# AlwinEsch/pvr.rtl.radiofm

Measured on AMD Instinct MI355X. Metric: IQ MS/s demodulated (whole node) + achieved HBM GB/s on FIR stage, higher is better.
Workload: dtype f32

## Files before the change

### pvr.rtl.radiofm_amd/csrc/fmd_batch.hip

```cpp
#include "../../include/fmd.h"

#include <hip/hip_runtime.h>
#include <hip/hip_ext.h>

#include <algorithm>
#include <chrono>
#include <cmath>
#include <cstdio>
#include <cstdlib>
#include <cstring>
#include <deque>
#include <functional>
#include <map>
#include <memory>
#include <mutex>
#include <string>
#include <utility>
#include <vector>

#include "fmd_design.hpp"
#include "fmd_groups.hpp"
#include "fmd_kernels.hip.h"
#include "fmd_receiver.hpp"

// ... 127 lines not shown
  unsigned min_samples = 0;
  int streams_sharing = 0;
  unsigned cpc = 1;
  unsigned Mmax = 0, Mstride = 0, Amax = 0, Rmax = 0;
  std::vector<unsigned> hb_nmax;
  unsigned lastM = 0, lastA = 0, lastR = 0;

  DevBuf<float2> lut, hist[2], demod[2], br[2], mix[2], rdsraw[2], rlpf[2], rs[2], alp[2];
  std::vector<DevBuf<float2>> hbbuf;
  DevBuf<float> if_coeff, rs_coeff, rds_lpf_taps, mf_taps2, audio_taps, ktab;
  DevBuf<float> rpll, rmf, tap_sync;
  DevBuf<double> sctab, sctab256;
  DevBuf<int> pidx;
  static constexpr unsigned kBrFront = 32;
  float2* brp(int q) const { return br[q].p + size_t(kBrFront) * CP; }
  unsigned rs_margin = 0, rs_row = 0;
  int rsr_R = 0, rsr_NW = 0;
  unsigned rsr_nbr = 0, rsr_nbm = 0;
  int rsr_rb = 0;
  DevBuf<float> rsr_tab;
  DevBuf<int> rsr_head, rsr_steps;
  int rsr_mode = -1;
  int n_cus = 256;
  struct HbfPlan
  {
    unsigned n_in = 0, S = 0;
    DevBuf<fmd::HbStep> steps;
    DevBuf<int> seg_first;
  };
  std::vector<std::unique_ptr<HbfPlan>> hbf_plans;
  DevBuf<float2> hbf_tail1, hbf_tail2;
  int hbf_mode = -1;
  static constexpr unsigned kOscH = 64;
  DevBuf<float2> osc_tab[4];
  HostBuf<float2> h_osc;
  Event osc_ev[8];
  bool osc_ev_used[8] = {};
  size_t h_osc_stride = 0;
  float osc_re = 1.0f, osc_im = 0.0f;
  bool osc_on = false;
  int dbg_nomix = 1;
  int dbg_fir_nt = 0;
  int dbg_serial_claim = 0;
  int dbg_hb4 = 1, dbg_ring4 = 1;
  int dbg_fir_ro = 2;
  int dbg_lpf_late = -1;
  double host_ms[4] = {0, 0, 0, 0};
  unsigned host_calls = 0;
  DevBuf<long long> serial_probe;
  int dbg_stage_mask = 63;
  DevBuf<float> fstate;
  DevBuf<int> istate;
  DevBuf<uint16_t> r_data;
  static constexpr int NSLOT = 8;
  static_assert(NSLOT == 8, "osc_ev / osc_ev_used above");
  DevBuf<fmd::RdsGroupRec> queue[NSLOT];
  DevBuf<unsigned> queue_counts;
  unsigned* qcount(int q) const { return queue_counts.p + q; }
  uint32_t drained_call[NSLOT] = {};
  HostBuf<unsigned> h_counts;
  HostBuf<fmd::RdsGroupRec> h_recs;
  unsigned queue_cap = 0;
  Event ev_drained[NSLOT];
  bool drained_pending[NSLOT] = {};
  static constexpr unsigned kExportCursors = 16;
  DevBuf<unsigned> export_cursor;
  unsigned export_seq = 0;
  fmd::ChannelState st{};
  std::vector<fmd::HbCoef> hbcoef;

  DevBuf<float> h_iq, h_audio;
  DevBuf<unsigned long long> pcm_clip;

  std::vector<std::unique_ptr<fmd::GroupDecoder>> gdec;

  int profiling = 0;
  int write_taps = 0;

  int concurrency = 1;
  hipStream_t s_fir = nullptr, s_ser = nullptr, s_post = nullptr, s_rds = nullptr, s_lpf = nullptr;
  struct LightJob
  {
    unsigned R = 0, A = 0, mf_g = 0, alpf_g = 0;
    unsigned rds_lpf_g = 0;
    const unsigned* org = nullptr;
    int q = 0, es = 0, sq = 0;
    bool events = true;
    bool lpf_here = false;
    int audio_after = -1;
    bool status_after_rds = false;
    hipEvent_t prev_aud = nullptr;
    uint32_t call_index = 0;
    void* d_audio = nullptr;
    int pcm = 0;
    size_t audio_stride = 0;
    hipEvent_t tl0 = nullptr, tl1 = nullptr;
  };
  std::vector<std::unique_ptr<fmd_batch>> subs;
  std::vector<unsigned> sub_ch0;
  bool owns_streams = true;
  hipEvent_t vheavy[2] = {nullptr, nullptr};
  hipEvent_t sched_prev2 = nullptr;
// ... 306 lines not shown
      independent = us < 250.0;
      for (int i = 0; i < have; i++)
        (void)hipStreamSynchronize(out[i]);
      (void)hipStreamSynchronize(nullptr);
    }
    if (independent)
      out[have++] = cand;
    else
      rejected.push_back(cand);
  }
  *n_sharing = 0;
  while (have < n && !rejected.empty())
  {
    out[have++] = rejected.back();
    rejected.pop_back();
    ++*n_sharing;
  }
  for (hipStream_t s : rejected)
    (void)hipStreamDestroy(s);
  return have == n ? 0 : -1;
}

fmd_batch::HbfPlan* hbf_plan(fmd_batch* b, unsigned n_in, unsigned S)
{
  for (auto& pl : b->hbf_plans)
    if (pl->n_in == n_in && pl->S == S)
      return pl.get();
  const fmd::Design& d = b->des;
  const int L1H = d.hb[1].len - 1, L2H = d.hb[2].len - 1, RING = fmd::HBF_RING;
  const int n0 = int(n_in + 1) / 2, n1 = (n0 + 1) / 2, n2 = (n1 + 1) / 2;
  std::vector<fmd::HbStep> steps;
  std::vector<int> first;
  const int per = (n2 + int(S) - 1) / int(S);
  for (int a = 0; a < n2; a += per)
  {
    first.push_back(int(steps.size()));
    const int e = std::min(n2, a + per);
    const bool last = e == n2;
    const int need1 = last ? n1 : 2 * (e - 1) + 1, need0 = last ? n0 : 2 * (need1 - 1) + 1;
    int d2 = a, d1 = std::max(0, 2 * a - L2H), d0 = std::max(0, 2 * d1 - L1H);
    while (d2 < e || d1 < need1 || d0 < need0)
    {
      const int a_hi = std::max(d0, std::min({d0 + 16, need0, 2 * d1 - L1H + RING}));
      const int b_hi = std::max(d1, std::min({d1 + 8, need1, a_hi > 0 ? (a_hi - 1) / 2 + 1 : 0, 2 * d2 - L2H + RING}));
      const int c_hi = std::max(d2, std::min({d2 + 4, e, b_hi > 0 ? (b_hi - 1) / 2 + 1 : 0}));
      if (a_hi == d0 && b_hi == d1 && c_hi == d2)
        return nullptr;
      steps.push_back(fmd::HbStep{d0, a_hi - d0, d1, b_hi - d1, d2, c_hi - d2, 0, 0});
      d0 = a_hi;
      d1 = b_hi;
      d2 = c_hi;
    }
    while ((steps.size() - size_t(first.back())) % 4)
      steps.push_back(fmd::HbStep{d0, 0, d1, 0, d2, 0, 0, 0});
  }
  first.push_back(int(steps.size()));
  std::unique_ptr<fmd_batch::HbfPlan> pl(new fmd_batch::HbfPlan);
  pl->n_in = n_in;
  pl->S = unsigned(first.size() - 1);
  if (pl->steps.alloc(steps.size()) || pl->seg_first.alloc(first.size()) ||
      upload(pl->steps.p, steps.data(), steps.size() * sizeof(fmd::HbStep)) ||
      upload(pl->seg_first.p, first.data(), first.size() * sizeof(int)))
    return nullptr;
  if (b->hbf_plans.size() >= 16)
  {
    (void)hipDeviceSynchronize();
    b->hbf_plans.erase(b->hbf_plans.begin());
  }
  b->hbf_plans.push_back(std::move(pl));
  return b->hbf_plans.back().get();
}

bool rsr_configure(fmd_batch* b, int form)
{
  static const int forms[3][2] = {{2, 8}, {4, 4}, {2, 4}};
  const fmd::Design& d = b->des;
  const int R = forms[form][0], NW = forms[form][1];
  const double step = double(d.rs_step);
  const unsigned per_step = unsigned(NW * R);
  const unsigned span = d.rs_order + 1u + unsigned(std::ceil((per_step - 1) * step)) + 1u;
  const unsigned nbr = (span - 1u + 7u) / 8u + 2u;
  const unsigned new_rows = unsigned(std::ceil(per_step * step)) + 8u;
  b->rsr_R = 0;
  if (nbr > 39u || new_rows > unsigned(fmd::RSR_ROWS))
    return false;
  b->rsr_R = R;
  b->rsr_NW = NW;
// ... 129 lines not shown
      auto t = fmd::make_tuner_lut(d.table_size, b->shifts[c]);
      std::copy(t.begin(), t.end(), &lut[size_t(2) * d.table_size * c]);
    }
  }

  b->Mmax = (FMD_MAX_BLOCK + d.D - 1) / d.D + 1;
  b->Mstride = (b->Mmax + 15u) & ~15u;
  b->Amax = unsigned(double(b->Mmax) / double(d.rs_step)) + 4;
  {
    unsigned n = b->Mmax;
    for (size_t s = 0; s < d.hb.size(); s++)
    {
      b->hb_nmax.push_back(n);
      n = (n + 1) / 2;
    }
    b->Rmax = n;
  }
  const unsigned T_lpf = unsigned(d.rds_lpf_taps.size());
  const unsigned T_mf = unsigned(d.rds_mf_taps.size());
  const unsigned T_alp = unsigned(d.lpf_taps.size());

  if (size_t(b->Mstride) * C * sizeof(float2) + 4096 >= (size_t(1) << 32) ||
      size_t(b->Mmax) * CP * sizeof(float2) >= (size_t(1) << 32))
    return fail(FMD_ERR_ARG, "too many channels for one batch at this sample rate (4 GB per row buffer): split the batch");
  int bad = 0;
  bad |= b->lut.alloc(size_t(d.table_size) * C);
  bad |= b->hist[0].alloc(size_t(d.if_order) * C);
  bad |= b->hist[1].alloc(size_t(d.if_order) * C);
  bad |= b->demod[0].alloc(size_t(b->Mstride) * C + fmd::DS);
  bad |= b->demod[1].alloc(size_t(b->Mstride) * C + fmd::DS);
  bad |= b->if_coeff.alloc(d.if_coeff.size() + 64);
  bad |= b->rs_coeff.alloc(d.rs_coeff.size());
  static_assert(fmd_batch::kBrFront >= 2 * fmd::RS_B, "front rows of br");
  bad |= b->br[0].alloc(size_t(fmd_batch::kBrFront + d.rs_order + b->Mmax + 8) * CP);
  bad |= b->br[1].alloc(size_t(fmd_batch::kBrFront + d.rs_order + b->Mmax + 8) * CP);
  if (d.hb.empty())
    return fail(FMD_ERR_ARG, "baseband rate too low for the RDS decimation chain");
  bad |= b->mix[0].alloc(size_t(d.hb[0].len - 1 + b->Mmax) * CP);
  bad |= b->mix[1].alloc(size_t(d.hb[0].len - 1 + b->Mmax) * CP);
  b->hbbuf.resize(d.hb.size() - 1);
  for (size_t s = 1; s < d.hb.size(); s++)
    bad |= b->hbbuf[s - 1].alloc(size_t(d.hb[s].len - 1 + b->hb_nmax[s]) * CP);
  if (d.hb.size() == 3)
  {
    bad |= b->hbf_tail1.alloc(size_t(d.hb[1].len - 1) * CP);
    bad |= b->hbf_tail2.alloc(size_t(d.hb[2].len - 1) * CP);
    for (auto& t : b->osc_tab)
      bad |= t.alloc(size_t(fmd_batch::kOscH) + b->Mmax + 8);
    b->h_osc_stride = size_t(fmd_batch::kOscH) + b->Mmax + 8;
    bad |= b->h_osc.alloc(fmd_batch::NSLOT * b->h_osc_stride);
    for (auto& e : b->osc_ev)
      bad |= e.create() != hipSuccess;
    const int h0 = (d.hb[0].len - 1) / 2, h1 = (d.hb[1].len - 1) / 2, h2 = (d.hb[2].len - 1) / 2;
    const bool chain_kind = h0 == 7 && ((h1 == 11 && h2 == 21) || (h1 == 9 && h2 == 17));
    b->osc_on = chain_kind && CP / 64 >= 64 && d.hb[0].len - 1 <= int(fmd_batch::kOscH);
  }
  bad |= b->rdsraw[0].alloc(size_t(T_lpf - 1 + b->Rmax) * CP);
  bad |= b->rdsraw[1].alloc(size_t(T_lpf - 1 + b->Rmax) * CP);
  bad |= b->rlpf[0].alloc(size_t(b->Rmax) * CP);
  bad |= b->rlpf[1].alloc(size_t(b->Rmax) * CP);
  bad |= b->rpll.alloc(size_t(T_mf - 1 + b->Rmax) * CP);
  bad |= b->rmf.alloc(size_t(b->Rmax) * CP);
  bad |= b->tap_sync.alloc(size_t(b->Rmax) * CP);
  bad |= b->rs[0].alloc(size_t(T_alp - 1 + b->Amax) * CP);
  bad |= b->rs[1].alloc(size_t(T_alp - 1 + b->Amax) * CP);
  bad |= b->alp[0].alloc(size_t(b->Amax) * CP);
  bad |= b->alp[1].alloc(size_t(b->Amax) * CP);
  bad |= b->rds_lpf_taps.alloc(T_lpf);
  bad |= b->mf_taps2.alloc(size_t(2) * T_mf);
  bad |= b->audio_taps.alloc(2 * size_t(T_alp));
  b->rs_margin = fmd::rs_table_margin(d.rs_step);
  b->rs_row = d.rs_order + 1 + 2 * b->rs_margin;
  bad |= b->ktab.alloc(size_t(b->Amax) * b->rs_row + 64);
  bad |= b->pidx.alloc(b->Amax);
  {
    hipDeviceProp_t prop{};
    if (hipGetDeviceProperties(&prop, device) == hipSuccess && prop.multiProcessorCount > 0)
      b->n_cus = prop.multiProcessorCount;
    size_t tab_floats = 0, head_ints = 0, step_ints = 0;
    for (int form = 0; form < 3; form++)
      if (rsr_configure(b.get(), form))
// ... 28 lines not shown
  }
  bad |= b->sctab.alloc(d.sincos_tab.size());
  bad |= b->sctab256.alloc(d.sincos_tab256.size());
  bad |= b->fstate.alloc(size_t(fmd::F_SLOTS) * CP);
  bad |= b->pcm_clip.alloc(CP);
  bad |= b->istate.alloc(size_t(fmd::I_SLOTS) * CP);
  bad |= b->r_data.alloc(size_t(4) * CP);
  b->queue_cap = std::max(4096u, 8u * C);
  for (int q = 0; q < fmd_batch::NSLOT; q++)
    bad |= b->queue[q].alloc(b->queue_cap);
  bad |= b->queue_counts.alloc(fmd_batch::NSLOT);
  bad |= b->h_counts.alloc(fmd_batch::NSLOT);
  bad |= b->export_cursor.alloc(fmd_batch::kExportCursors);
  if (bad)
    return fail(FMD_ERR_DEVICE, std::string("device allocation failed: ") + hipGetErrorString(hipGetLastError()));

  bad |= upload(b->lut.p, lut.data(), lut.size() * sizeof(float));
  bad |= upload(b->if_coeff.p, d.if_coeff.data(), d.if_coeff.size() * sizeof(float));
  bad |= upload(b->rs_coeff.p, d.rs_coeff.data(), d.rs_coeff.size() * sizeof(float));
  bad |= upload(b->rds_lpf_taps.p, d.rds_lpf_taps.data(), T_lpf * sizeof(float));
  bad |= upload(b->audio_taps.p, d.lpf_taps.data(), T_alp * sizeof(float));
  bad |= upload(b->audio_taps.p + T_alp, d.lpf_taps.data(), T_alp * sizeof(float));
  bad |= upload(b->sctab.p, d.sincos_tab.data(), d.sincos_tab.size() * sizeof(double));
  bad |= upload(b->sctab256.p, d.sincos_tab256.data(), d.sincos_tab256.size() * sizeof(double));
  bad |= upload(b->mf_taps2.p, d.rds_mf_taps.data(), T_mf * sizeof(float));
  for (const auto& h : d.hb)
  {
    fmd::HbCoef hc{};
    for (int i = 0; i < h.len; i++)
      hc.c[i] = h.coef[size_t(i)];
    for (int j = 0; 2 * j < h.len && j < 28; j++)
      hc.e[j] = hc.c[2 * j];
    b->hbcoef.push_back(hc);
  }
  if (b->h_err.alloc(2, hipHostMallocMapped | hipHostMallocCoherent))
    return fail(FMD_ERR_DEVICE, "host-mapped error word allocation failed");
  if (b->h_status.alloc(size_t(fmd::HS_WORDS) * CP, hipHostMallocMapped | hipHostMallocCoherent))
    return fail(FMD_ERR_DEVICE, "host-mapped status snapshot allocation failed");
  if (b->d_status.alloc(size_t(fmd::HS_WORDS) * CP))
    return fail(FMD_ERR_DEVICE, "status record allocation failed");
  if (b->org.alloc(size_t(2) * CP) || b->d_edits.alloc(size_t(fmd_batch::NSLOT) * 2 * C))
    return fail(FMD_ERR_DEVICE, "device allocation of the channel edit state failed");
  if (b->h_edits.alloc(size_t(fmd_batch::NSLOT) * 2 * C))
    return fail(FMD_ERR_DEVICE, "page-locked staging allocation failed");
  for (auto& e : b->edit_ev)
    HIPCHK(e.create());
  bind_state(b.get());
  if (!b->st.err || !b->st.hs)
    return fail(FMD_ERR_DEVICE, "host-mapped memory has no device address");
  bad |= init_signal_state(b.get());
  if (bad)
    return fail(FMD_ERR_DEVICE, "upload of constants failed");
  if (do_reset(b.get()))
    return fail(FMD_ERR_DEVICE, "state reset failed");

  b->gdec.resize(C);
  if (shell)
  {
    b->owns_streams = false;
    b->s_fir = shell->s_fir;
    b->s_ser = shell->s_ser;
    b->s_post = shell->s_post;
    b->s_rds = shell->s_rds;
    b->s_lpf = shell->s_lpf;
    b->streams_sharing = shell->streams_sharing;
  }
// ... 1903 lines not shown
```

### pvr.rtl.radiofm_amd/csrc/fmd_batch_process.inc.hpp

```cpp
namespace
{

fmd::DemodConsts demod_consts(const fmd::Design& d)
{
  fmd::DemodConsts k{};
  k.pll_alpha = d.pll_alpha;
  k.pll_beta = d.pll_beta;
  k.nco_hl = d.nco_hl;
  k.nco_ll = d.nco_ll;
  k.demod_gain = d.demod_gain;
  k.p_minfreq = d.p_minfreq;
  k.p_maxfreq = d.p_maxfreq;
  k.p_b0 = d.p_b0;
  k.p_a1 = d.p_a1;
  k.p_a2 = d.p_a2;
  k.p_lf_b0 = d.p_lf_b0;
  k.p_lf_b1 = d.p_lf_b1;
  k.p_minsignal = d.p_minsignal;
  k.p_lock_delay = d.p_lock_delay;
  k.osc_cos = d.rds_osc_cos;
  k.osc_sin = d.rds_osc_sin;
  return k;
}

// ... 310 lines not shown
    }
    evset = &b->ev[size_t(b->prof_calls) * (ST_COUNT + 1)];
  }
  auto timed = [&](int i) -> hipEvent_t { return evset && b->profiling == 1 && !serial_mode ? evset[i].e : nullptr; };
  auto mark = [&](int i) {
    if (evset && b->profiling >= 2 && i > 1)
      note(hipEventRecord(evset[i], sF));
  };

  bool hb_all_normal = d.hb.size() <= 3;
  for (size_t s = 0; s < d.hb.size(); s++)
    hb_all_normal = hb_all_normal && hb_mode[s] == HB_NORMAL && d.hb[s].len != 11 && !d.hb[s].cic;
  fmd_batch::HbfPlan* hbf_pl = nullptr;
  int hbf_kind = -1;
  if (hb_all_normal && d.hb.size() == 3 && b->hbf_mode != 0 && (b->hbf_mode == 1 || CP / 64 >= 64))
  {
    const int h0 = (d.hb[0].len - 1) / 2, h1 = (d.hb[1].len - 1) / 2, h2 = (d.hb[2].len - 1) / 2;
    hbf_kind = (h0 == 7 && h1 == 11 && h2 == 21) ? 0 : (h0 == 7 && h1 == 9 && h2 == 17) ? 1 : -1;
    if (hbf_kind >= 0)
    {
      const unsigned groups = CP / 64;
      const unsigned ncu = unsigned(b->n_cus) - ((b->serial_exclusive && !serial_mode) ? (groups + 1) / 2 : 0u);
      const unsigned S = std::max(1u, std::min({8u, (2u * ncu + groups / 2u) / groups, R / 32u}));
      hbf_pl = hbf_plan(b, hb_in[0], S);
    }
  }
  const bool nomix = hbf_pl != nullptr && b->osc_on && b->dbg_nomix != 0;
  const unsigned osc_slot = ci & 3u;
  float osc_re = b->osc_re, osc_im = b->osc_im;
  if (b->osc_on)
  {
    if (b->osc_ev_used[es])
      note(hipEventSynchronize(b->osc_ev[es]));
    float2* h = b->h_osc.p + size_t(es) * b->h_osc_stride;
    const float2* hp = b->h_osc.p + size_t((ci + fmd_batch::NSLOT - 1) % fmd_batch::NSLOT) * b->h_osc_stride;
    std::memcpy(h, hp + b->lastM, fmd_batch::kOscH * sizeof(float2));
    const float oc = d.rds_osc_cos, os = d.rds_osc_sin;
    float2* o = h + fmd_batch::kOscH;
    for (unsigned t = 0; t < M; t++)
    {
      const float x = osc_re * oc - osc_im * os;
      const float y = osc_im * oc + osc_re * os;
      const float gn = float(1.95 - double(osc_re * osc_re + osc_im * osc_im));
      osc_re = gn * x;
      osc_im = gn * y;
      o[t] = make_float2(x, y);
    }
    note(hipMemcpyAsync(b->osc_tab[osc_slot].p, h, (fmd_batch::kOscH + M) * sizeof(float2), hipMemcpyHostToDevice, sF));
    note(hipEventRecord(b->osc_ev[es], sF));
    b->osc_ev_used[es] = true;
  }
  if (b->map_on && b->map_dirty)
  {
    if (b->walk_ev_used[es])
      note(hipEventSynchronize(b->walk_ev[es]));
    uint2* h = b->h_walk.p + size_t(es) * C;
    build_walk(b, h);
    note(hipMemcpyAsync(b->d_walk.p, h, C * sizeof(uint2), hipMemcpyHostToDevice, sF));
    note(hipEventRecord(b->walk_ev[es], sF));
    b->walk_ev_used[es] = true;
    b->map_dirty = false;
  }

  const bool input_pending = serial_mode ? false : hipStreamQuery(stream) != hipSuccess;
  (void)hipGetLastError();
  if (input_pending)
  {
    signal(ce[fmd_batch::EV_IN], stream);
    after(sF, ce[fmd_batch::EV_IN]);
  }
  if (have_prev2)
  {
    if (stage_mask != 63u)
      after(sF, pe2[fmd_batch::EV_SER]);
    after(sF, pe2[fmd_batch::EV_HEAVY]);
  }
  if (b->sched_prev2 && !serial_mode)
    after(sF, b->sched_prev2);
  {
    const std::function<void(int)> markfn = [&](int i) {
      mark(i);
// ... 73 lines not shown
  hipStream_t sLPr = lpf_late ? b->s_lpf : sR;
  hipStream_t sLPa = lpf_late ? b->s_lpf : sA;
  const unsigned per_step = unsigned(std::max(b->rsr_NW * b->rsr_R, 1));
  const unsigned rs_steps = (A + per_step - 1) / per_step;
  const bool ring = b->rsr_R != 0 && b->rsr_mode != 0 &&
                    (b->rsr_mode == 1 || (CP / 64 >= 64 && rs_steps >= 24 && per_step >= 16));
  bool rs_planned = false;
  auto rs_plan = [&](hipStream_t s) {
    if (!ring || rs_planned)
      return;
    rs_planned = true;
    auto go = [&](auto plan) {
      hipLaunchKernelGGL(plan, dim3(rs_steps * b->rsr_NW), dim3(64), 0, s, b->rs_coeff.p, d.rs_order, p, pstep, A,
                         b->rsr_rb, b->rsr_nbr, b->rsr_tab.p, b->rsr_nbm, b->rsr_head.p, b->rsr_steps.p);
    };
    if (b->rsr_R == 4)
      go(&fmd::k_rs_plan<4, 4>);
    else if (b->rsr_NW == 8)
      go(&fmd::k_rs_plan<2, 8>);
    else
      go(&fmd::k_rs_plan<2, 4>);
  };
  auto rds_heavy = [&]() {
    after(sR, ce[fmd_batch::EV_SER]);
    if (nomix && sR != sA && ci > 1)
      after(sR, b->cev[(ci + fmd_batch::NSLOT - 1) % fmd_batch::NSLOT][fmd_batch::EV_ROLL]);
    post_delay(sR);
    bool chain_done = false;
    if (hbf_pl)
    {
      fmd_batch::HbfPlan* pl = hbf_pl;
      const unsigned groups = CP / 64;
      const unsigned L0H = unsigned(d.hb[0].len - 1);
      const unsigned n0 = (hb_in[0] + 1) / 2, n1 = (n0 + 1) / 2;
      const float2* in0 = nomix ? (const float2*)(b->brp(q) + size_t(Hbb - L0H) * CP) : (const float2*)b->mix[q].p;
      const float2* osc = nomix ? (const float2*)(b->osc_tab[osc_slot].p + (fmd_batch::kOscH - L0H)) : nullptr;
      auto kern = hbf_kind == 0 ? (nomix ? &fmd::k_halfband_chain<7, 11, 21, true> : &fmd::k_halfband_chain<7, 11, 21, false>)
                                : (nomix ? &fmd::k_halfband_chain<7, 9, 17, true> : &fmd::k_halfband_chain<7, 9, 17, false>);
      launch(kern, dim3(groups, pl->S), dim3(64, 4), 0, sR, timed(6), timed(7), in0, b->hbbuf[0].p, b->hbbuf[1].p,
             b->rdsraw[q].p, T_lpf - 1, b->hbf_tail1.p, b->hbf_tail2.p, b->hbcoef[0], b->hbcoef[1], b->hbcoef[2],
             pl->steps.p, pl->seg_first.p, hb_in[0], n0, n1, C, CP, osc, 0u);
      if (nomix)
        mix_tail = [&, L0H]() {
          hipLaunchKernelGGL(fmd::k_mix_tail, rgrid(L0H), rt, 0, sR,
                             (const float2*)(b->brp(q) + size_t(Hbb + hb_in[0] - L0H) * CP),
                             (const float2*)(b->osc_tab[osc_slot].p + fmd_batch::kOscH + hb_in[0] - L0H),
                             b->mix[q ^ 1].p, L0H, CP);
        };
      else
        roll_later(b->mix[q].p, b->mix[q ^ 1].p, L0H, hb_in[0]);
      roll_later(b->hbf_tail1.p, b->hbbuf[0].p, unsigned(d.hb[1].len - 1), 0u);
      roll_later(b->hbf_tail2.p, b->hbbuf[1].p, unsigned(d.hb[2].len - 1), 0u);
      chain_done = true;
    }
    if (!chain_done)
    {
      const float2* in = b->mix[q].p;
      for (size_t s = 0; s < d.hb.size(); s++)
      {
        const unsigned n_out =
            (d.hb[s].cic || d.hb[s].len == 11 || hb_mode[s] == HB_PASS) ? hb_in[s] / 2 : (hb_in[s] + 1) / 2;
        const bool last = (s + 1 == d.hb.size());
        float2* outp = last ? b->rdsraw[q].p : b->hbbuf[s].p;
        const unsigned Hout = last ? (T_lpf - 1) : unsigned(d.hb[s + 1].len - 1);
        const int hb4 = b->dbg_hb4;
        const unsigned Hs = unsigned(d.hb[s].len - 1);
        float2* const hist_dst = s == 0 ? b->mix[q ^ 1].p : b->hbbuf[s - 1].p;
        if (hb_mode[s] == HB_PASS)
        {
          hipLaunchKernelGGL(fmd::k_hb_pass, rgrid(n_out), rt, 0, sR, in, Hs, outp, Hout, n_out, CP);
          if (s == 0)
            hipLaunchKernelGGL(fmd::k_roll<float2>, rgrid(Hs), rt, 0, sR, b->mix[q].p, b->mix[q ^ 1].p, Hs, 0u, CP);
          in = outp;
          continue;
        }
        if (d.hb[s].cic)
          hipLaunchKernelGGL(fmd::k_cic3, dim3(CP / 64, (n_out + 3) / 4), dim3(64, 4), 0, sR, in, outp, n_out, C, CP,
                             Hout);
        else if (d.hb[s].len == 11)
// ... 248 lines not shown
```

### pvr.rtl.radiofm_amd/csrc/fmd_k_rds.hip.h

```cpp
#pragma once

#include "fmd_k_common.hip.h"

namespace fmd
{

struct HbCoef
{
  float c[52];
  float e[28];
};

#ifndef FMD_HB_R
#define FMD_HB_R 4
#endif
constexpr int HB_R = FMD_HB_R;

__global__ __launch_bounds__(256) void k_halfband(const float2* __restrict__ in,
                                                  float2* __restrict__ out, unsigned n_out, int L,
                                                  HbCoef hc, unsigned C, unsigned CP, unsigned Hout)
{
  const unsigned c = blockIdx.x * 64 + threadIdx.x;
  const unsigned wy = (unsigned)__builtin_amdgcn_readfirstlane((int)threadIdx.y);
  const unsigned k0 = (blockIdx.y * blockDim.y + wy) * HB_R;
// ... 153 lines not shown
    const float2 x = p[(size_t)(half + m) * step];
#pragma unroll
    for (int r = m; r < RR; r++)
      rf_acc(acc[r], hc.e[half + m - r], x);
  }
#pragma unroll
  for (int r = 0; r < RR; r++)
  {
    const float2 x = p[(size_t)(2 * r + half) * CP];
    rf_acc(acc[r], hc.c[half], x);
    out[(size_t)(Hout + k0 + r) * CP + c] = acc[r];
  }
}

__global__ __launch_bounds__(256) void k_halfband4(const float2* __restrict__ in,
                                                   float2* __restrict__ out, unsigned n_out, int L,
                                                   HbCoef hc, unsigned C, unsigned CP, unsigned Hout)
{
  const unsigned c = blockIdx.x * 64 + threadIdx.x;
  const unsigned wy = (unsigned)__builtin_amdgcn_readfirstlane((int)threadIdx.y);
  const unsigned k0 = (blockIdx.y * blockDim.y + wy) * 4;
  if (c >= C || k0 >= n_out)
    return;
  const int half = (L - 1) / 2;
  switch (min(4u, n_out - k0))
  {
    case 4: hb_group<4>(in, out, k0, half, hc, c, CP, Hout); break;
    case 3: hb_group<3>(in, out, k0, half, hc, c, CP, Hout); break;
    case 2: hb_group<2>(in, out, k0, half, hc, c, CP, Hout); break;
    default: hb_group<1>(in, out, k0, half, hc, c, CP, Hout); break;
  }
}

__global__ void k_mix_tail(const float2* __restrict__ br_last, const float2* __restrict__ osc_last,
                           float2* __restrict__ dst, unsigned H, unsigned CP)
{
  const unsigned c = blockIdx.x * blockDim.x + threadIdx.x;
  if (c >= CP)
    return;
  for (unsigned r = blockIdx.y; r < H; r += gridDim.y)
  {
    const float v = br_last[(size_t)r * CP + c].x;
    const float2 o = osc_last[r];
    const float zero = 0.0f;
    dst[(size_t)r * CP + c] = make_float2((v * o.x) - (zero * o.y), (v * o.y) + (zero * o.x));
  }
}

struct HbStep
{
  int a_lo, a_n, b_lo, b_n, c_lo, c_n;
  int pad0, pad1;
};
constexpr int HBF_RING = 64;

template <int RR, int HALF, class LD>
__device__ __forceinline__ void hb_rows(LD ld, const HbCoef& hc, float2 (&acc)[RR])
{
  static_assert(HALF >= RR, "half-band group");
#pragma unroll
  for (int u = 0; u < RR + HALF; u++)
  {
    const float2 x = ld(2 * u);
#pragma unroll
    for (int r = 0; r < RR; r++)
    {
      const int j = u - r;
      if (j == 0)
      {
        acc[r] = rf_mul(hc.e[0], x);
        rf_acc(acc[r], hc.e[0], x);
      }
      else if (j > 0 && j <= HALF)
        rf_acc(acc[r], hc.e[j], x);
    }
  }
#pragma unroll
  for (int r = 0; r < RR; r++)
    rf_acc(acc[r], hc.c[HALF], ld(2 * r + HALF));
}

template <int H0, int H1, int H2, bool OSC = false>
__global__ __launch_bounds__(256) void k_halfband_chain(
    const float2* __restrict__ mix, const float2* __restrict__ hist1, const float2* __restrict__ hist2,
    float2* __restrict__ out, unsigned Hout, float2* __restrict__ tail1, float2* __restrict__ tail2,
    HbCoef hc0, HbCoef hc1, HbCoef hc2, const HbStep* __restrict__ steps, const int* __restrict__ seg_first,
    unsigned n_in, unsigned n0, unsigned n1, unsigned C, unsigned CP, const float2* __restrict__ osc,
    unsigned prio)
{
  wave_prio(prio);
  __shared__ float2 ring1[HBF_RING][64];
  __shared__ float2 ring2[HBF_RING][64];
  constexpr int L1H = 2 * H1, L2H = 2 * H2;
  static_assert(L1H + 34 <= HBF_RING && L2H + 18 <= HBF_RING, "ring size");
  const unsigned lane = threadIdx.x;
  const int w = __builtin_amdgcn_readfirstlane((int)threadIdx.y);
  const unsigned c0 = blockIdx.x * 64 + lane;
  const bool live = c0 < C;
  const unsigned c = live ? c0 : C - 1;
  const int s_begin = seg_first[blockIdx.y], s_end = seg_first[blockIdx.y + 1];
  if (s_begin >= s_end)
    return;
  const float2* __restrict__ mp = mix + c;
  const size_t rowstride = CP;
  constexpr int NA = 4 + H0 + 4;
  constexpr int NSET = 4;
  float2 xs[NSET][NA];
  auto fetch_a = [&](float2 (&x)[NA], const HbStep& st) {
    const int k0 = st.a_lo + 4 * w;
    const int last = 2 * H0 + (int)n_in - 1;
#pragma unroll
    for (int u = 0; u < 4 + H0; u++)
      x[u] = mp[(size_t)min(2 * k0 + 2 * u, last) * rowstride];
#pragma unroll
    for (int r = 0; r < 4; r++)
      x[4 + H0 + r] = mp[(size_t)min(2 * k0 + 2 * r + H0, last) * rowstride];
  };
  {
    const HbStep f = steps[s_begin];
    if (2 * f.b_lo - L1H < 0)
      for (int i = w; i < L1H; i += 4)
        ring1[(i - L1H) & (HBF_RING - 1)][lane] = hist1[(size_t)i * rowstride + c];
    if (2 * f.c_lo - L2H < 0)
      for (int i = w; i < L2H; i += 4)
        ring2[(i - L2H) & (HBF_RING - 1)][lane] = hist2[(size_t)i * rowstride + c];
#pragma unroll
    for (int k = 0; k < NSET - 1; k++)
      fetch_a(xs[k], steps[s_begin + k]);
  }
  __syncthreads();
  HbStep cur = steps[s_begin], far = steps[min(s_begin + NSET - 1, s_end - 1)];
  auto step = [&](int s, float2 (&x)[NA], float2 (&xn)[NA]) {
    const HbStep st = cur;
    const HbStep cur_next = steps[min(s + 1, s_end - 1)], far_next = steps[min(s + NSET, s_end - 1)];
    fetch_a(xn, far);
    {
      const int k0 = st.a_lo + 4 * w;
      const int nr = min(4, st.a_lo + st.a_n - k0);
      if (nr > 0)
      {
        float2 acc[4];
        hb_rows<4, H0>(
            [&](int row) {
              const float2 v = (row & 1) ? x[4 + H0 + (row - H0) / 2] : x[row / 2];
              if constexpr (!OSC)
                return v;
              else
              {
                const float2 o = osc[min(2 * k0 + row, 2 * H0 + (int)n_in - 1)];
                const float zero = 0.0f;
                return make_float2((v.x * o.x) - (zero * o.y), (v.x * o.y) + (zero * o.x));
              }
            },
            hc0, acc);
#pragma unroll
        for (int r = 0; r < 4; r++)
          if (r < nr)
          {
            const int i0 = k0 + r;
            ring1[i0 & (HBF_RING - 1)][lane] = acc[r];
            if (live && i0 >= (int)n0 - L1H)
              tail1[(size_t)(i0 - ((int)n0 - L1H)) * rowstride + c] = acc[r];
          }
      }
    }
    lds_barrier();
    {
      const int k0 = st.b_lo + 2 * w;
      const int nr = min(2, st.b_lo + st.b_n - k0);
      if (nr > 0)
      {
        float2 acc[2];
        hb_rows<2, H1>([&](int row) { return ring1[(2 * k0 + row - L1H) & (HBF_RING - 1)][lane]; }, hc1, acc);
#pragma unroll
        for (int r = 0; r < 2; r++)
          if (r < nr)
          {
            const int i1 = k0 + r;
            ring2[i1 & (HBF_RING - 1)][lane] = acc[r];
            if (live && i1 >= (int)n1 - L2H)
              tail2[(size_t)(i1 - ((int)n1 - L2H)) * rowstride + c] = acc[r];
          }
      }
    }
    lds_barrier();
    {
      const int k0 = st.c_lo + w;
      if (k0 < st.c_lo + st.c_n)
      {
        float2 acc[1];
        hb_rows<1, H2>([&](int row) { return ring2[(2 * k0 + row - L2H) & (HBF_RING - 1)][lane]; }, hc2, acc);
        if (live)
          out[(size_t)(Hout + (unsigned)k0) * rowstride + c] = acc[0];
      }
    }
    cur = cur_next;
    far = far_next;
  };
  for (int s = s_begin; s < s_end; s += NSET)
  {
#pragma unroll
    for (int k = 0; k < NSET; k++)
      step(s + k, xs[k], xs[(k + NSET - 1) % NSET]);
  }
}

__device__ __forceinline__ int ring_wave_g0(const unsigned* __restrict__ origin, unsigned c, unsigned C, unsigned g0,
                                            int T, unsigned* lane_g0)
{
  const unsigned o_lane = c < C ? origin[c] : 0u;
  const unsigned o0 = (unsigned)__builtin_amdgcn_readfirstlane((int)o_lane);
  const unsigned o = c < C ? o_lane : o0;
  *lane_g0 = (g0 + (unsigned)T - o) % (unsigned)T;
  if (__ballot(o != o0) != 0ull)
    return -1;
  return (int)((g0 + (unsigned)T - o0) % (unsigned)T);
}

template <typename E>
__device__ __forceinline__ E ring_one_mixed(const E* __restrict__ now, size_t stride, unsigned a0, int T,
                                            const float* __restrict__ taps)
{
  const E* __restrict__ p = now - a0 * stride;
  E acc = rf_mul(taps[a0], *p);
  unsigned a = a0;
  for (int s = 1; s < T; s++)
  {
    const bool wrap = a + 1 == (unsigned)T;
    a = wrap ? 0u : a + 1;
    p = wrap ? now : p - stride;
    rf_acc(acc, taps[a], *p);
  }
  return acc;
}

template <typename E, bool ORG>
// ... 508 lines not shown
```

Baseline: 293,600.

## Pack half-band step records and use buffer loads, packed FMA taps in chain kernel

Step records for the fused half-band decimation chain are packed into a single word holding the counts, tail flags, prefetch distance and a last-step flag. Tail buffer pointers move into a header after each segment. Kernel arguments shrink to one scalar tap table that is applied with v_pk_mul_f32, and the oscillator table gets a precomputed second half so mixing becomes a packed multiply-add. Global reads and stores now go through raw buffer loads with fixed offsets (row buffers gain slack rows so reads past the end stay in bounds), and ring reads use contiguous LDS fast paths. The aim is to cut scalar register pressure, address arithmetic and per-step loads in the inner loop, at the cost of inline asm, bit-packing limits that make the plan builder return failure, and extra padded allocations.

```diff
diff --git a/pvr.rtl.radiofm_amd/csrc/fmd_batch.hip b/pvr.rtl.radiofm_amd/csrc/fmd_batch.hip
--- a/pvr.rtl.radiofm_amd/csrc/fmd_batch.hip
+++ b/pvr.rtl.radiofm_amd/csrc/fmd_batch.hip
@@ -183,8 +183,8 @@
   DevBuf<float2> hbf_tail1, hbf_tail2;
   int hbf_mode = -1;
   static constexpr unsigned kOscH = 64;
-  DevBuf<float2> osc_tab[4];
-  HostBuf<float2> h_osc;
+  DevBuf<fmd::HbOsc> osc_tab[4];
+  HostBuf<fmd::HbOsc> h_osc;
   Event osc_ev[8];
   bool osc_ev_used[8] = {};
   size_t h_osc_stride = 0;
@@ -219,6 +219,7 @@
   unsigned export_seq = 0;
   fmd::ChannelState st{};
   std::vector<fmd::HbCoef> hbcoef;
+  fmd::HbChainTaps hb_taps{};
 
   DevBuf<float> h_iq, h_audio;
   DevBuf<unsigned long long> pcm_clip;
@@ -591,13 +592,27 @@
   std::vector<fmd::HbStep> steps;
   std::vector<int> first;
   const int per = (n2 + int(S) - 1) / int(S);
+  fmd::HbTails tails{};
+  tails.tail1 = b->hbf_tail1.p;
+  tails.tail2 = b->hbf_tail2.p;
+  tails.first1 = n0 - L1H;
+  tails.first2 = n1 - L2H;
   for (int a = 0; a < n2; a += per)
   {
     first.push_back(int(steps.size()));
+    const size_t f = steps.size();
     const int e = std::min(n2, a + per);
     const bool last = e == n2;
     const int need1 = last ? n1 : 2 * (e - 1) + 1, need0 = last ? n0 : 2 * (need1 - 1) + 1;
     int d2 = a, d1 = std::max(0, 2 * a - L2H), d0 = std::max(0, 2 * d1 - L1H);
+    auto push = [&](int an, int bn, int cn) {
+      unsigned n = unsigned(an) | unsigned(bn) << 5 | unsigned(cn) << 9;
+      if (an > 0 && d0 + an > tails.first1)
+        n |= fmd::HBF_TAIL0;
+      if (bn > 0 && d1 + bn > tails.first2)
+        n |= fmd::HBF_TAIL1;
+      steps.push_back(fmd::HbStep{d0, d1, d2, n});
+    };
     while (d2 < e || d1 < need1 || d0 < need0)
     {
       const int a_hi = std::max(d0, std::min({d0 + 16, need0, 2 * d1 - L1H + RING}));
@@ -605,13 +620,29 @@
       const int c_hi = std::max(d2, std::min({d2 + 4, e, b_hi > 0 ? (b_hi - 1) / 2 + 1 : 0}));
       if (a_hi == d0 && b_hi == d1 && c_hi == d2)
         return nullptr;
-      steps.push_back(fmd::HbStep{d0, a_hi - d0, d1, b_hi - d1, d2, c_hi - d2, 0, 0});
+      push(a_hi - d0, b_hi - d1, c_hi - d2);
       d0 = a_hi;
       d1 = b_hi;
       d2 = c_hi;
     }
-    while ((steps.size() - size_t(first.back())) % 4)
-      steps.push_back(fmd::HbStep{d0, 0, d1, 0, d2, 0, 0, 0});
+    while ((steps.size() - f) % fmd::HBF_NSET)
+      push(0, 0, 0);
+    const size_t g = steps.size();
+    for (size_t i = f; i < g; i++)
+    {
+      const int far = steps[std::min(i + size_t(fmd::HBF_NSET - 1), g - 1)].a_lo - steps[i].a_lo;
+      if (far < 0 || far > 63 || g - i > 1023)
+        return nullptr;
+      steps[i].n |= unsigned(far) << fmd::HBF_FAR_SHIFT;
+      if (steps[i].n & (fmd::HBF_TAIL0 | fmd::HBF_TAIL1))
+        steps[i].n |= unsigned(g - i) << fmd::HBF_TAILS_SHIFT;
+    }
+    steps[g - 1].n |= fmd::HBF_LAST;
+    fmd::HbStep hdr[2];
+    static_assert(sizeof(hdr) == sizeof(tails), "HbTails in the place of two records");
+    std::memcpy(hdr, &tails, sizeof(tails));
+    steps.push_back(hdr[0]);
+    steps.push_back(hdr[1]);
   }
   first.push_back(int(steps.size()));
   std::unique_ptr<fmd_batch::HbfPlan> pl(new fmd_batch::HbfPlan);
@@ -807,12 +838,12 @@
   bad |= b->if_coeff.alloc(d.if_coeff.size() + 64);
   bad |= b->rs_coeff.alloc(d.rs_coeff.size());
   static_assert(fmd_batch::kBrFront >= 2 * fmd::RS_B, "front rows of br");
-  bad |= b->br[0].alloc(size_t(fmd_batch::kBrFront + d.rs_order + b->Mmax + 8) * CP);
-  bad |= b->br[1].alloc(size_t(fmd_batch::kBrFront + d.rs_order + b->Mmax + 8) * CP);
+  bad |= b->br[0].alloc(size_t(fmd_batch::kBrFront + d.rs_order + b->Mmax + 8 + fmd::HBF_SLACK) * CP);
+  bad |= b->br[1].alloc(size_t(fmd_batch::kBrFront + d.rs_order + b->Mmax + 8 + fmd::HBF_SLACK) * CP);
   if (d.hb.empty())
     return fail(FMD_ERR_ARG, "baseband rate too low for the RDS decimation chain");
-  bad |= b->mix[0].alloc(size_t(d.hb[0].len - 1 + b->Mmax) * CP);
-  bad |= b->mix[1].alloc(size_t(d.hb[0].len - 1 + b->Mmax) * CP);
+  bad |= b->mix[0].alloc(size_t(d.hb[0].len - 1 + b->Mmax + fmd::HBF_SLACK) * CP);
+  bad |= b->mix[1].alloc(size_t(d.hb[0].len - 1 + b->Mmax + fmd::HBF_SLACK) * CP);
   b->hbbuf.resize(d.hb.size() - 1);
   for (size_t s = 1; s < d.hb.size(); s++)
     bad |= b->hbbuf[s - 1].alloc(size_t(d.hb[s].len - 1 + b->hb_nmax[s]) * CP);
@@ -821,7 +852,7 @@
     bad |= b->hbf_tail1.alloc(size_t(d.hb[1].len - 1) * CP);
     bad |= b->hbf_tail2.alloc(size_t(d.hb[2].len - 1) * CP);
     for (auto& t : b->osc_tab)
-      bad |= t.alloc(size_t(fmd_batch::kOscH) + b->Mmax + 8);
+      bad |= t.alloc(size_t(fmd_batch::kOscH) + b->Mmax + 8 + fmd::HBF_SLACK);
     b->h_osc_stride = size_t(fmd_batch::kOscH) + b->Mmax + 8;
     bad |= b->h_osc.alloc(fmd_batch::NSLOT * b->h_osc_stride);
     for (auto& e : b->osc_ev)
@@ -916,6 +947,19 @@
     for (int j = 0; 2 * j < h.len && j < 28; j++)
       hc.e[j] = hc.c[2 * j];
     b->hbcoef.push_back(hc);
+  }
+  if (d.hb.size() == 3)
+  {
+    float* t = &b->hb_taps.p[0].x;
+    int k = 0;
+    for (const auto& h : d.hb)
+    {
+      const int half = (h.len - 1) / 2;
+      for (int j = 0; j <= half && k < fmd::HBF_TAPS; j++)
+        t[k++] = h.coef[size_t(2 * j)];
+      if (k < fmd::HBF_TAPS)
+        t[k++] = h.coef[size_t(half)];
+    }
   }
   if (b->h_err.alloc(2, hipHostMallocMapped | hipHostMallocCoherent))
     return fail(FMD_ERR_DEVICE, "host-mapped error word allocation failed");
diff --git a/pvr.rtl.radiofm_amd/csrc/fmd_batch_process.inc.hpp b/pvr.rtl.radiofm_amd/csrc/fmd_batch_process.inc.hpp
--- a/pvr.rtl.radiofm_amd/csrc/fmd_batch_process.inc.hpp
+++ b/pvr.rtl.radiofm_amd/csrc/fmd_batch_process.inc.hpp
@@ -366,11 +366,12 @@
   {
     if (b->osc_ev_used[es])
       note(hipEventSynchronize(b->osc_ev[es]));
-    float2* h = b->h_osc.p + size_t(es) * b->h_osc_stride;
-    const float2* hp = b->h_osc.p + size_t((ci + fmd_batch::NSLOT - 1) % fmd_batch::NSLOT) * b->h_osc_stride;
-    std::memcpy(h, hp + b->lastM, fmd_batch::kOscH * sizeof(float2));
+    fmd::HbOsc* h = b->h_osc.p + size_t(es) * b->h_osc_stride;
+    const fmd::HbOsc* hp = b->h_osc.p + size_t((ci + fmd_batch::NSLOT - 1) % fmd_batch::NSLOT) * b->h_osc_stride;
+    std::memcpy(h, hp + b->lastM, fmd_batch::kOscH * sizeof(fmd::HbOsc));
     const float oc = d.rds_osc_cos, os = d.rds_osc_sin;
-    float2* o = h + fmd_batch::kOscH;
+    fmd::HbOsc* o = h + fmd_batch::kOscH;
+    const volatile float zero = 0.0f;
     for (unsigned t = 0; t < M; t++)
     {
       const float x = osc_re * oc - osc_im * os;
@@ -378,9 +379,11 @@
       const float gn = float(1.95 - double(osc_re * osc_re + osc_im * osc_im));
       osc_re = gn * x;
       osc_im = gn * y;
-      o[t] = make_float2(x, y);
-    }
-    note(hipMemcpyAsync(b->osc_tab[osc_slot].p, h, (fmd_batch::kOscH + M) * sizeof(float2), hipMemcpyHostToDevice, sF));
+      o[t].xy = make_float2(x, y);
+      o[t].z = make_float2(-(zero * y), zero * x);
+    }
+    note(hipMemcpyAsync(b->osc_tab[osc_slot].p, h, (fmd_batch::kOscH + M) * sizeof(fmd::HbOsc), hipMemcpyHostToDevice,
+                        sF));
     note(hipEventRecord(b->osc_ev[es], sF));
     b->osc_ev_used[es] = true;
   }
@@ -520,19 +523,18 @@
       fmd_batch::HbfPlan* pl = hbf_pl;
       const unsigned groups = CP / 64;
       const unsigned L0H = unsigned(d.hb[0].len - 1);
-      const unsigned n0 = (hb_in[0] + 1) / 2, n1 = (n0 + 1) / 2;
       const float2* in0 = nomix ? (const float2*)(b->brp(q) + size_t(Hbb - L0H) * CP) : (const float2*)b->mix[q].p;
-      const float2* osc = nomix ? (const float2*)(b->osc_tab[osc_slot].p + (fmd_batch::kOscH - L0H)) : nullptr;
+      const fmd::HbOsc* osc = nomix ? b->osc_tab[osc_slot].p + (fmd_batch::kOscH - L0H) : nullptr;
       auto kern = hbf_kind == 0 ? (nomix ? &fmd::k_halfband_chain<7, 11, 21, true> : &fmd::k_halfband_chain<7, 11, 21, false>)
                                 : (nomix ? &fmd::k_halfband_chain<7, 9, 17, true> : &fmd::k_halfband_chain<7, 9, 17, false>);
       launch(kern, dim3(groups, pl->S), dim3(64, 4), 0, sR, timed(6), timed(7), in0, b->hbbuf[0].p, b->hbbuf[1].p,
-             b->rdsraw[q].p, T_lpf - 1, b->hbf_tail1.p, b->hbf_tail2.p, b->hbcoef[0], b->hbcoef[1], b->hbcoef[2],
-             pl->steps.p, pl->seg_first.p, hb_in[0], n0, n1, C, CP, osc, 0u);
+             b->rdsraw[q].p + size_t(T_lpf - 1) * CP, b->hb_taps, (const fmd::HbStep*)pl->steps.p,
+             (const int*)pl->seg_first.p, C, CP, osc, 0u);
       if (nomix)
         mix_tail = [&, L0H]() {
           hipLaunchKernelGGL(fmd::k_mix_tail, rgrid(L0H), rt, 0, sR,
                              (const float2*)(b->brp(q) + size_t(Hbb + hb_in[0] - L0H) * CP),
-                             (const float2*)(b->osc_tab[osc_slot].p + fmd_batch::kOscH + hb_in[0] - L0H),
+                             (const fmd::HbOsc*)(b->osc_tab[osc_slot].p + fmd_batch::kOscH + hb_in[0] - L0H),
                              b->mix[q ^ 1].p, L0H, CP);
         };
       else
diff --git a/pvr.rtl.radiofm_amd/csrc/fmd_k_rds.hip.h b/pvr.rtl.radiofm_amd/csrc/fmd_k_rds.hip.h
--- a/pvr.rtl.radiofm_amd/csrc/fmd_k_rds.hip.h
+++ b/pvr.rtl.radiofm_amd/csrc/fmd_k_rds.hip.h
@@ -209,7 +209,13 @@
   }
 }
 
-__global__ void k_mix_tail(const float2* __restrict__ br_last, const float2* __restrict__ osc_last,
+struct HbOsc
+{
+  float2 xy;
+  float2 z;
+};
+
+__global__ void k_mix_tail(const float2* __restrict__ br_last, const HbOsc* __restrict__ osc_last,
                            float2* __restrict__ dst, unsigned H, unsigned CP)
 {
   const unsigned c = blockIdx.x * blockDim.x + threadIdx.x;
@@ -218,7 +224,7 @@
   for (unsigned r = blockIdx.y; r < H; r += gridDim.y)
   {
     const float v = br_last[(size_t)r * CP + c].x;
-    const float2 o = osc_last[r];
+    const float2 o = osc_last[r].xy;
     const float zero = 0.0f;
     dst[(size_t)r * CP + c] = make_float2((v * o.x) - (zero * o.y), (v * o.y) + (zero * o.x));
   }
@@ -226,72 +232,171 @@
 
 struct HbStep
 {
-  int a_lo, a_n, b_lo, b_n, c_lo, c_n;
+  int a_lo, b_lo, c_lo;
+  unsigned n;
+};
+constexpr unsigned HBF_TAIL0 = 1u << 12, HBF_TAIL1 = 1u << 13, HBF_LAST = 1u << 14;
+constexpr int HBF_FAR_SHIFT = 16, HBF_TAILS_SHIFT = 22;
+struct HbTails
+{
+  float2 *tail1, *tail2;
+  int first1, first2;
   int pad0, pad1;
 };
+static_assert(sizeof(HbTails) == 2 * sizeof(HbStep), "the step list's header");
+typedef float HbPair __attribute__((ext_vector_type(2)));
+__device__ __forceinline__ void hb_store_global(float2* p, float2 v)
+{
+  HbPair x;
+  x[0] = v.x;
+  x[1] = v.y;
+  *(__attribute__((address_space(1))) HbPair*)p = x;
+}
 constexpr int HBF_RING = 64;
-
-template <int RR, int HALF, class LD>
-__device__ __forceinline__ void hb_rows(LD ld, const HbCoef& hc, float2 (&acc)[RR])
+constexpr int HBF_NSET = 4;
+
+constexpr int HBF_SLACK = 32;
+
+constexpr int HBF_TAPS = 45;
+struct HbChainTaps
+{
+  float2 p[(HBF_TAPS + 1) / 2];
+};
+
+__device__ __forceinline__ float2 hb_tap_mul(const HbChainTaps& tp, int j, float2 x)
+{
+  float2 r;
+  const float2 pr = tp.p[j / 2];
+  if (j % 2 == 0)
+    asm("v_pk_mul_f32 %0, %1, %2 op_sel_hi:[1,0]" : "=v"(r) : "v"(x), "s"(pr));
+  else
+    asm("v_pk_mul_f32 %0, %1, %2 op_sel:[0,1]" : "=v"(r) : "v"(x), "s"(pr));
+  return r;
+}
+__device__ __forceinline__ float2 hb_osc_mul(float2 v, HbOsc o)
+{
+  float2 m, r;
+  asm("v_pk_mul_f32 %0, %1, %2 op_sel_hi:[0,1]" : "=v"(m) : "v"(v), "s"(o.xy));
+  asm("v_pk_add_f32 %0, %1, %2" : "=v"(r) : "v"(m), "s"(o.z));
+  return r;
+}
+__device__ __forceinline__ float2 hb_add(float2 a, float2 b) { return make_float2(a.x + b.x, a.y + b.y); }
+
+template <int RR, int HALF, int T>
+__device__ __forceinline__ void hb_rows(const float2* xe, const float2* xc, const HbChainTaps& tp, float2 (&acc)[RR])
 {
   static_assert(HALF >= RR, "half-band group");
 #pragma unroll
   for (int u = 0; u < RR + HALF; u++)
   {
-    const float2 x = ld(2 * u);
+    const float2 x = xe[u];
 #pragma unroll
     for (int r = 0; r < RR; r++)
     {
       const int j = u - r;
       if (j == 0)
       {
-        acc[r] = rf_mul(hc.e[0], x);
-        rf_acc(acc[r], hc.e[0], x);
+        acc[r] = hb_tap_mul(tp, T, x);
+        acc[r] = hb_add(acc[r], hb_tap_mul(tp, T, x));
       }
       else if (j > 0 && j <= HALF)
-        rf_acc(acc[r], hc.e[j], x);
+        acc[r] = hb_add(acc[r], hb_tap_mul(tp, T + j, x));
     }
   }
 #pragma unroll
   for (int r = 0; r < RR; r++)
-    rf_acc(acc[r], hc.c[HALF], ld(2 * r + HALF));
+    acc[r] = hb_add(acc[r], hb_tap_mul(tp, T + HALF + 1, xc[r]));
+}
+
+template <int RR, int HALF>
+__device__ __forceinline__ void ring_rows(const float2 (*ring)[64], int row0, unsigned lane, float2 (&xe)[RR + HALF],
+                                          float2 (&xc)[RR])
+{
+  constexpr int SPAN = 2 * (RR + HALF - 1) + 1;
+  const int slot = row0 & (HBF_RING - 1);
+  if (slot + SPAN <= HBF_RING)
+  {
+    const float2* p = &ring[slot][lane];
+#pragma unroll
+    for (int u = 0; u < RR + HALF; u++)
+      xe[u] = p[2 * u * 64];
+#pragma unroll
+    for (int r = 0; r < RR; r++)
+      xc[r] = p[(2 * r + HALF) * 64];
+  }
+  else
+  {
+    const char* base = reinterpret_cast<const char*>(&ring[0][0]);
+    const unsigned a = (unsigned)slot * 512u + lane * 8u;
+    auto at = [&](int row) { return *reinterpret_cast<const float2*>(base + ((a + (unsigned)row * 512u) & 0x7fffu)); };
+#pragma unroll
+    for (int u = 0; u < RR + HALF; u++)
+      xe[u] = at(2 * u);
+#pragma unroll
+    for (int r = 0; r < RR; r++)
+      xc[r] = at(2 * r + HALF);
+  }
+}
+
+template <int RR>
+__device__ __forceinline__ void ring_put(float2 (*ring)[64], int k0, int nr, unsigned lane, const float2 (&acc)[RR])
+{
+  const int slot = k0 & (HBF_RING - 1);
+  if (nr == RR && slot <= HBF_RING - RR)
+  {
+    float2* p = &ring[slot][lane];
+#pragma unroll
+    for (int r = 0; r < RR; r++)
+      p[r * 64] = acc[r];
+  }
+  else
+  {
+#pragma unroll
+    for (int r = 0; r < RR; r++)
+      if (r < nr)
+        ring[(k0 + r) & (HBF_RING - 1)][lane] = acc[r];
+  }
 }
 
 template <int H0, int H1, int H2, bool OSC = false>
 __global__ __launch_bounds__(256) void k_halfband_chain(
     const float2* __restrict__ mix, const float2* __restrict__ hist1, const float2* __restrict__ hist2,
-    float2* __restrict__ out, unsigned Hout, float2* __restrict__ tail1, float2* __restrict__ tail2,
-    HbCoef hc0, HbCoef hc1, HbCoef hc2, const HbStep* __restrict__ steps, const int* __restrict__ seg_first,
-    unsigned n_in, unsigned n0, unsigned n1, unsigned C, unsigned CP, const float2* __restrict__ osc,
-    unsigned prio)
+    float2* __restrict__ out, HbChainTaps tp, const HbStep* __restrict__ steps, const int* __restrict__ seg_first,
+    unsigned C, unsigned CP, const HbOsc* __restrict__ osc, unsigned prio)
 {
   wave_prio(prio);
   __shared__ float2 ring1[HBF_RING][64];
   __shared__ float2 ring2[HBF_RING][64];
   constexpr int L1H = 2 * H1, L2H = 2 * H2;
   static_assert(L1H + 34 <= HBF_RING && L2H + 18 <= HBF_RING, "ring size");
+  static_assert((H0 + 2) + (H1 + 2) + (H2 + 2) <= HBF_TAPS, "tap table");
+  static_assert(H0 % 2 == 1 && H1 % 2 == 1 && H2 % 2 == 1, "the centre rows are odd rows");
+  constexpr int T1 = H0 + 2, T2 = T1 + H1 + 2;
   const unsigned lane = threadIdx.x;
-  const int w = __builtin_amdgcn_readfirstlane((int)threadIdx.y);
+  const int w = __builtin_amdgcn_readfirstlane((int)threadIdx.y), w4 = 4 * w;
   const unsigned c0 = blockIdx.x * 64 + lane;
-  const bool live = c0 < C;
-  const unsigned c = live ? c0 : C - 1;
+  const unsigned c = c0 < C ? c0 : C - 1;
   const int s_begin = seg_first[blockIdx.y], s_end = seg_first[blockIdx.y + 1];
   if (s_begin >= s_end)
     return;
-  const float2* __restrict__ mp = mix + c;
   const size_t rowstride = CP;
-  constexpr int NA = 4 + H0 + 4;
-  constexpr int NSET = 4;
-  float2 xs[NSET][NA];
-  auto fetch_a = [&](float2 (&x)[NA], const HbStep& st) {
-    const int k0 = st.a_lo + 4 * w;
-    const int last = 2 * H0 + (int)n_in - 1;
-#pragma unroll
-    for (int u = 0; u < 4 + H0; u++)
-      x[u] = mp[(size_t)min(2 * k0 + 2 * u, last) * rowstride];
-#pragma unroll
-    for (int r = 0; r < 4; r++)
-      x[4 + H0 + r] = mp[(size_t)min(2 * k0 + 2 * r + H0, last) * rowstride];
+  constexpr int NE = 4 + H0, NA = NE + 4;
+  constexpr int NSET = HBF_NSET;
+  using Row = float2;
+  Row xs[NSET][NA];
+  const char* const gb = reinterpret_cast<const char*>(mix);
+  const unsigned row_bytes = CP * (unsigned)sizeof(float2), lane_off = c * (unsigned)sizeof(float2);
+  auto row_of = [](int i) { return i < NE ? 2 * i : 2 * (i - NE) + H0; };
+  auto fetch_a = [&](Row (&x)[NA], int a_lo) {
+    const char* rp = gb + (uint64_t)(unsigned)(2 * (a_lo + w4)) * row_bytes;
+    const __amdgpu_buffer_rsrc_t rs = __builtin_amdgcn_make_buffer_rsrc(const_cast<char*>(rp), 0, -1, 0x00020000);
+#pragma unroll
+    for (int i = 0; i < NA; i++)
+    {
+      const unsigned off = lane_off + (unsigned)row_of(i) * row_bytes;
+      const auto v = __builtin_amdgcn_raw_buffer_load_b64(rs, off, 0, 0);
+      x[i] = make_float2(__uint_as_float(v[0]), __uint_as_float(v[1]));
+    }
   };
   {
     const HbStep f = steps[s_begin];
@@ -303,82 +408,96 @@
         ring2[(i - L2H) & (HBF_RING - 1)][lane] = hist2[(size_t)i * rowstride + c];
 #pragma unroll
     for (int k = 0; k < NSET - 1; k++)
-      fetch_a(xs[k], steps[s_begin + k]);
+      fetch_a(xs[k], steps[s_begin + k].a_lo);
   }
   __syncthreads();
-  HbStep cur = steps[s_begin], far = steps[min(s_begin + NSET - 1, s_end - 1)];
-  auto step = [&](int s, float2 (&x)[NA], float2 (&xn)[NA]) {
+  const HbStep* __restrict__ sp = steps + s_begin;
+  HbStep cur = sp[0];
+  auto step = [&](int k, Row (&x)[NA], Row (&xn)[NA]) {
     const HbStep st = cur;
-    const HbStep cur_next = steps[min(s + 1, s_end - 1)], far_next = steps[min(s + NSET, s_end - 1)];
-    fetch_a(xn, far);
-    {
-      const int k0 = st.a_lo + 4 * w;
-      const int nr = min(4, st.a_lo + st.a_n - k0);
+    cur = sp[k + 1];
+    int wq = w4;
+    asm volatile("" : "+s"(wq));
+    fetch_a(xn, st.a_lo + (int)((st.n >> HBF_FAR_SHIFT) & 63u));
+    {
+      const int k0 = st.a_lo + wq;
+      const int nr = min(4, st.a_lo + (int)(st.n & 31u) - k0);
       if (nr > 0)
       {
         float2 acc[4];
-        hb_rows<4, H0>(
-            [&](int row) {
-              const float2 v = (row & 1) ? x[4 + H0 + (row - H0) / 2] : x[row / 2];
-              if constexpr (!OSC)
-                return v;
-              else
-              {
-                const float2 o = osc[min(2 * k0 + row, 2 * H0 + (int)n_in - 1)];
-                const float zero = 0.0f;
-                return make_float2((v.x * o.x) - (zero * o.y), (v.x * o.y) + (zero * o.x));
-              }
-            },
-            hc0, acc);
-#pragma unroll
-        for (int r = 0; r < 4; r++)
-          if (r < nr)
+        if constexpr (!OSC)
+          hb_rows<4, H0, 0>(x, x + NE, tp, acc);
+        else
+        {
+          float2 xm[NA];
+          const HbOsc* __restrict__ op = osc + 2 * k0;
+#pragma unroll
+          for (int i = 0; i < NA; i++)
           {
-            const int i0 = k0 + r;
-            ring1[i0 & (HBF_RING - 1)][lane] = acc[r];
-            if (live && i0 >= (int)n0 - L1H)
-              tail1[(size_t)(i0 - ((int)n0 - L1H)) * rowstride + c] = acc[r];
+          {
+            xm[i] = hb_osc_mul(x[i], op[row_of(i)]);
+            if (i % 4 == 3)
+              __builtin_amdgcn_sched_barrier(0);
           }
+          }
+          hb_rows<4, H0, 0>(xm, xm + NE, tp, acc);
+        }
+        ring_put<4>(ring1, k0, nr, lane, acc);
+        if (st.n & HBF_TAIL0)
+        {
+          const HbTails t = *reinterpret_cast<const HbTails*>(sp + k + (st.n >> HBF_TAILS_SHIFT));
+#pragma unroll
+          for (int r = 0; r < 4; r++)
+            if (r < nr && k0 + r >= t.first1)
+              hb_store_global(t.tail1 + ((size_t)(k0 + r - t.first1) * CP + c), acc[r]);
+        }
       }
     }
     lds_barrier();
     {
-      const int k0 = st.b_lo + 2 * w;
-      const int nr = min(2, st.b_lo + st.b_n - k0);
+      const int k0 = st.b_lo + (wq >> 1);
+      const int nr = min(2, st.b_lo + (int)((st.n >> 5) & 15u) - k0);
       if (nr > 0)
       {
-        float2 acc[2];
-        hb_rows<2, H1>([&](int row) { return ring1[(2 * k0 + row - L1H) & (HBF_RING - 1)][lane]; }, hc1, acc);
-#pragma unroll
-        for (int r = 0; r < 2; r++)
-          if (r < nr)
-          {
-            const int i1 = k0 + r;
-            ring2[i1 & (HBF_RING - 1)][lane] = acc[r];
-            if (live && i1 >= (int)n1 - L2H)
-              tail2[(size_t)(i1 - ((int)n1 - L2H)) * rowstride + c] = acc[r];
-          }
+        float2 xe[2 + H1], xc[2], acc[2];
+        ring_rows<2, H1>(ring1, 2 * k0 - L1H, lane, xe, xc);
+        hb_rows<2, H1, T1>(xe, xc, tp, acc);
+        ring_put<2>(ring2, k0, nr, lane, acc);
+        if (st.n & HBF_TAIL1)
+        {
+          const HbTails t = *reinterpret_cast<const HbTails*>(sp + k + (st.n >> HBF_TAILS_SHIFT));
+#pragma unroll
+          for (int r = 0; r < 2; r++)
+            if (r < nr && k0 + r >= t.first2)
+              hb_store_global(t.tail2 + ((size_t)(k0 + r - t.first2) * CP + c), acc[r]);
+        }
       }
     }
     lds_barrier();
     {
-      const int k0 = st.c_lo + w;
-      if (k0 < st.c_lo + st.c_n)
+      const int k0 = st.c_lo + (wq >> 2);
+      if (k0 < st.c_lo + (int)((st.n >> 9) & 7u))
       {
-        float2 acc[1];
-        hb_rows<1, H2>([&](int row) { return ring2[(2 * k0 + row - L2H) & (HBF_RING - 1)][lane]; }, hc2, acc);
-        if (live)
-          out[(size_t)(Hout + (unsigned)k0) * rowstride + c] = acc[0];
+        float2 xe[1 + H2], xc[1], acc[1];
+        ring_rows<1, H2>(ring2, 2 * k0 - L2H, lane, xe, xc);
+        hb_rows<1, H2, T2>(xe, xc, tp, acc);
+        {
+          char* op = reinterpret_cast<char*>(out) + (uint64_t)(unsigned)k0 * row_bytes;
+          typedef unsigned hb_u2 __attribute__((ext_vector_type(2)));
+          hb_u2 v;
+          v[0] = __float_as_uint(acc[0].x);
+          v[1] = __float_as_uint(acc[0].y);
+          __builtin_amdgcn_raw_buffer_store_b64(v, __builtin_amdgcn_make_buffer_rsrc(op, 0, -1, 0x00020000), lane_off, 0, 0);
+        }
       }
     }
-    cur = cur_next;
-    far = far_next;
+    return (st.n & HBF_LAST) != 0u;
   };
-  for (int s = s_begin; s < s_end; s += NSET)
+  for (bool last = false; !last; sp += NSET)
   {
 #pragma unroll
     for (int k = 0; k < NSET; k++)
-      step(s + k, xs[k], xs[(k + NSET - 1) % NSET]);
+      last = step(k, xs[k], xs[(k + NSET - 1) % NSET]);
   }
 }
 
```

Measured after the change: 300,300 (median of 6 runs). +2.3%, better.
